# nihalsid/single-view-3d-reconstruction

Measured on AMD Instinct MI355X. Metric: query-points/sec fwd+bwd (128^3 grid, 50k pts), higher is better.
Workload: dtype f32

## Files before the change

include/svr_hip.h:

```cpp
#ifndef SVR_HIP_H
#define SVR_HIP_H

#include <stdint.h>

#ifdef __cplusplus
extern "C" {
#endif

#define SVR_OK 0
#define SVR_E_BADARG (-1)
#define SVR_E_BADSHAPE (-2)
#define SVR_E_ALIGN (-3)
#define SVR_E_UNSUPPORTED (-4)
#define SVR_E_IO (-5)
#define SVR_E_NOTFOUND (-6)

#define SVR_MAX_LEVELS 6

int svr_version(void);
const char *svr_last_error(void);

typedef struct svr_pull_plan {
  const uint32_t *keys;
  const void *recs;
// ... 183 lines not shown
int64_t svr_conv3d_bwd_data_f16x3_workspace(int32_t Ci, int32_t Co);
int svr_conv3d_k3_bwd_data_f16x3(const float *dout, const float *W, float *din, int32_t B, int32_t D,
                                 int32_t H, int32_t Wd, int32_t Ci, int32_t Co, int epilogue,
                                 const float *mask, const uint32_t *amax_dout, uint32_t *amax_din,
                                 void *workspace, void *stream);
int svr_conv3d_k3_bwd_weight_f16x3(const float *in, const float *dout, float *dW, float *db, int32_t B,
                                   int32_t D, int32_t H, int32_t W, int32_t Ci, int32_t Co, int32_t param_layout,
                                   const uint32_t *amax_dout, void *workspace, void *stream);
#define SVR_CONV_FWD_F16X3 0
#define SVR_CONV_BWD_DATA_F16X3S 1
#define SVR_CONV_BWD_DATA_BF16X3 2
#define SVR_CONV_FWD_BF16X6 3
int svr_conv3d_k3_variant(int32_t op, int32_t B, int32_t D, int32_t H, int32_t Wd, int32_t Ci, int32_t Co, int32_t *ck,
                          int32_t *tn, int32_t *vt, int32_t *persistent, int64_t *workgroup_rows);

int64_t svr_bn_stats_workspace(int64_t rows, int32_t C);
int svr_bn_stats(const float *x, double *stats, int64_t rows , int32_t C,
                 void *workspace, void *stream);
int svr_bn_stats_finalize(const float *x, double *stats, const float *gamma, const float *beta, float *running_mean,
                          float *running_var, float *scale_shift, float *mean_f32, int64_t rows, int32_t C,
                          float eps, float momentum, void *workspace, void *stream);
int svr_bn_finalize_parts(const double *part, int32_t blocks, double *stats, const float *gamma, const float *beta,
                          float *running_mean, float *running_var, float *scale_shift, float *mean_f32, int64_t rows,
                          int32_t C, float eps, float momentum, void *stream);
int svr_bn_finalize(const double *stats, const float *gamma, const float *beta, float *running_mean,
                    float *running_var, float *scale_shift, float *mean_f32, int64_t rows,
                    int32_t C, float eps, float momentum, int training, void *stream);
int svr_bn_apply_pool(const float *x, const float *scale_shift, float *y, float *pooled,
                      uint8_t *argmax, int32_t B, int32_t D, int32_t H, int32_t W, int32_t C,
                      void *stream);
// ... 119 lines not shown
```

single-view-3d-reconstruction_amd/_lib.py:

```python
import ctypes as C
import os

_HERE = os.path.dirname(os.path.abspath(__file__))
LIB_PATH = os.path.join(_HERE, "lib", "libsvr_hip.so")

SVR_MAX_LEVELS = 6
EPI_NONE, EPI_BIAS, EPI_BIAS_RELU, EPI_MASK = 0, 1, 2, 3

P = C.c_void_p
I32, I64, F32 = C.c_int32, C.c_int64, C.c_float


class Conv2dDesc(C.Structure):
    _fields_ = [("src0", P), ("src1", P), ("B", I32), ("H", I32), ("W", I32), ("C0", I32), ("C1", I32), ("k", I32),
                ("stride", I32), ("act", I32), ("upsample", I32)]


class PullPlan(C.Structure):
    _fields_ = [("keys", P), ("recs", P), ("heads", P), ("n_items", I64)]


class Level(C.Structure):
    _fields_ = [("vol", P), ("gvol", P), ("C", I32), ("D", I32), ("H", I32), ("W", I32), ("col", I32), ("order", P),
                ("item_order", P), ("plan", C.POINTER(PullPlan))]
# ... 70 lines not shown
    "svr_conv3d_fwd_f16x3_stats_blocks": (I32, [I32, I32, I32, I32, I32, I32]),
    "svr_conv3d_k3_fwd_f16x3_stats": (C.c_int, [P, P, P, P, P, I32, I32, I32, I32, I32, I32, C.c_int, P, P]),
    "svr_conv3d_bwd_data_bf16x3_workspace": (I64, [I32, I32]),
    "svr_conv3d_k3_bwd_data_bf16x3": (C.c_int, [P, P, P, I32, I32, I32, I32, I32, I32, C.c_int, P, P, P]),
    "svr_conv3d_c1_fwd_stats_workspace": (I64, [I32, I32, I32, I32, I32]),
    "svr_conv3d_c1_fwd_stats": (C.c_int, [P, P, P, P, P, I32, I32, I32, I32, I32, C.c_int, P, P]),
    "svr_conv3d_k3_bwd_weight_workspace": (I64, [I32, I32, I32, I32, I32, I32]),
    "svr_conv3d_k3_bwd_weight": (C.c_int, [P, P, P, P, I32, I32, I32, I32, I32, I32, P, P]),
    "svr_conv3d_k3_bwd_weight_bf16x3_workspace": (I64, [I32, I32, I32, I32, I32, I32]),
    "svr_conv3d_k3_bwd_weight_bf16x3": (C.c_int, [P, P, P, P, I32, I32, I32, I32, I32, I32, P, P]),
    "svr_conv3d_k3_bwd_weight_bf16x3_param": (C.c_int, [P, P, P, P, I32, I32, I32, I32, I32, I32, P, P]),
    "svr_conv3d_bwd_data_f16x3_workspace": (I64, [I32, I32]),
    "svr_conv3d_k3_bwd_data_f16x3": (C.c_int, [P, P, P, I32, I32, I32, I32, I32, I32, C.c_int, P, P, P, P, P]),
    "svr_conv3d_k3_bwd_weight_f16x3": (C.c_int, [P, P, P, P, I32, I32, I32, I32, I32, I32, I32, P, P, P]),
    "svr_conv3d_k3_variant": (C.c_int, [I32, I32, I32, I32, I32, I32, I32, P, P, P, P, P]),
    "svr_bn_stats_workspace": (I64, [I64, I32]),
    "svr_bn_stats": (C.c_int, [P, P, I64, I32, P, P]),
    "svr_bn_stats_finalize": (C.c_int, [P, P, P, P, P, P, P, P, I64, I32, F32, F32, P, P]),
    "svr_bn_finalize_parts": (C.c_int, [P, I32, P, P, P, P, P, P, P, I64, I32, F32, F32, P]),
    "svr_bn_finalize": (C.c_int, [P, P, P, P, P, P, P, I64, I32, F32, F32, C.c_int, P]),
    "svr_bn_apply_pool": (C.c_int, [P, P, P, P, P, I32, I32, I32, I32, I32, P]),
    "svr_bn_bwd_reduce": (C.c_int, [P, P, P, P, P, P, P, I32, I32, I32, I32, I32, P, P]),
    "svr_bn_bwd_apply": (C.c_int, [P, P, P, P, P, P, P, P, P, P, P, I32, I32, I32, I32, I32, C.c_int, P, P]),
    "svr_stage1_supported": (I32, [I32, I32, I32, I32, I32]),
    "svr_stage1_workspace": (I64, [I32, I32, I32, I32]),
    "svr_stage1_fwd": (C.c_int, [P, P, P, P, P, P, P, P, P, P, P, P, P, I32, I32, I32, I32, I32, F32, F32, C.c_int, C.c_int, P, P]),
    "svr_stage1_bwd": (C.c_int, [P, P, P, P, P, P, P, P, P, P, P, P, P, P, I32, I32, I32, I32, I32, C.c_int, C.c_int, P, P]),
    "svr_conv2d_im2col": (C.c_int, [C.POINTER(Conv2dDesc), P, P]),
    "svr_conv2d_col2im": (C.c_int, [C.POINTER(Conv2dDesc), P, P, P, P, P]),
    "svr_conv2d_small_supported": (C.c_int, [I32, I32, I32]),
# ... 74 lines not shown
```

single-view-3d-reconstruction_amd/build.py:

```python
import os
import subprocess
import sys

HERE = os.path.dirname(os.path.abspath(__file__))
CSRC = os.path.join(HERE, "csrc")
INCLUDE = os.path.join(os.path.dirname(HERE), "include")
LIBDIR = os.path.join(HERE, "lib")
LIB = os.path.join(LIBDIR, "libsvr_hip.so")

SOURCES = {
    "capi.cpp": [],
    "gather.hip": ["-ffp-contract=off"],
    "gather_fc0.hip": ["-ffp-contract=off"],
    "sort.hip": [],
    "gemm.hip": [],
    "gemm_bf16x3.hip": [],
    "gemm_bf16x6.hip": [],
    "gemm_f16x3.hip": [],
    "conv3d.hip": [],
    "conv3d_bf16.hip": [],
    "conv3d_bwdw_bf16.hip": [],
    "bn_pool.hip": [],
    "stage1.hip": [],
    "projection.hip": ["-ffp-contract=off"],
    "bf16_path.hip": ["-ffp-contract=off"],
    "mesh_occupancy.hip": ["-ffp-contract=off"],
    "marching_cubes.hip": ["-ffp-contract=off"],
    "mesh_eval.hip": ["-ffp-contract=off"],
    "sample_io.hip": [],
    "conv2d.hip": [],
    "conv2d_igemm.hip": [],
}
COMMON = ["-O3", "-fPIC", "--offload-arch=gfx950", "-munsafe-fp-atomics", "-std=c++17", "-I" + INCLUDE, "-I" + CSRC,
          "-Rpass-analysis=kernel-resource-usage"]


# ... 80 lines not shown
```

single-view-3d-reconstruction_amd/csrc/conv3d_bf16.hip:

```cpp
#include "common.h"
#include <cstdlib>
#include "f16x3.h"

using namespace svr;

namespace {

typedef __bf16 bf16x8 __attribute__((ext_vector_type(8)));
typedef __bf16 bf16x2 __attribute__((ext_vector_type(2)));
typedef float f32x16 __attribute__((ext_vector_type(16)));

struct ConvShape {
  int B, D, H, W, Ci, Co;
};

constexpr int BRZ = 4, BRY = 4, BRX = 8;
constexpr int HLZ = BRZ + 2, HLY = BRY + 2, HLX = BRX + 2, HLV = HLZ * HLY * HLX;

__device__ __forceinline__ void split2(float x0, float x1, uint32_t &hi, uint32_t &mid) {
  f32x2 v = {x0, x1};
  bf16x2 h = __builtin_convertvector(v, bf16x2);
  hi = __builtin_bit_cast(uint32_t, h);
  f32x2 r = {x0 - __uint_as_float(hi << 16), x1 - __uint_as_float(hi & 0xffff0000u)};
  bf16x2 m = __builtin_convertvector(r, bf16x2);
  mid = __builtin_bit_cast(uint32_t, m);
}

__device__ __forceinline__ void split3(float x0, float x1, uint32_t &hi, uint32_t &mid, uint32_t &lo) {
  split2(x0, x1, hi, mid);
  f32x2 r = {(x0 - __uint_as_float(hi << 16)) - __uint_as_float(mid << 16),
             (x1 - __uint_as_float(hi & 0xffff0000u)) - __uint_as_float(mid & 0xffff0000u)};
  bf16x2 l = __builtin_convertvector(r, bf16x2);
  lo = __builtin_bit_cast(uint32_t, l);
}

constexpr int HP = 12;
template <int SL>
__device__ __forceinline__ int slot_dw(int row, int sub) {
  static_assert(SL == 2 || SL == 4, "16- or 32-channel chunks");
  const int g = SL == 2 ? (row >> 3) & 1 : (row >> 2) & 3;
  return (row * SL + (sub ^ g)) * 4;
// ... 3 lines not shown

__device__ __forceinline__ bf16x8 read_frag(const uint32_t *p) {
  union { uint4 q; bf16x8 v; } f;
  f.q = *reinterpret_cast<const uint4 *>(p);
  return f.v;
}

__device__ __forceinline__ f16x8 read_frag_h(const uint32_t *p) {
  union { uint4 q; f16x8 v; } f;
  f.q = *reinterpret_cast<const uint4 *>(p);
  return f.v;
}

__global__ void pack_fwd_planes_f16_kernel(const float *__restrict__ W, const uint32_t *__restrict__ amax,
                                           uint16_t *__restrict__ p0, uint16_t *__restrict__ p1, int Ci, int Co) {
  int idx = blockIdx.x * blockDim.x + threadIdx.x;
  if (idx >= 27 * Co * (Ci / 2)) return;
  const int ci = (idx % (Ci / 2)) * 2;
  const int co = (idx / (Ci / 2)) % Co;
  const int tap = idx / ((Ci / 2) * Co);
  const float sc = w_scale(amax[0], false);
  const float w0 = W[((size_t)co * Ci + ci) * 27 + tap] * sc, w1 = W[((size_t)co * Ci + ci + 1) * 27 + tap] * sc;
  const uint32_t hi = pack_f16(w0, w1);
  const f32x2 h = unpack_f16(hi);
  const size_t o = ((size_t)tap * Co + co) * Ci + ci;
  *reinterpret_cast<uint32_t *>(p0 + o) = hi;
  *reinterpret_cast<uint32_t *>(p1 + o) = pack_f16(w0 - h.x, w1 - h.y);
}

__global__ void pack_bwd_planes_kernel(const float *__restrict__ W, uint16_t *__restrict__ hi, uint16_t *__restrict__ mid,
                                       int Ci, int Co) {
  int idx = blockIdx.x * blockDim.x + threadIdx.x;
  if (idx >= 27 * Ci * (Co / 2)) return;
  const int co = (idx % (Co / 2)) * 2;
  const int ci = (idx / (Co / 2)) % Ci;
  const int tp = idx / ((Co / 2) * Ci);
  uint32_t h, m;
  split2(W[((size_t)co * Ci + ci) * 27 + (26 - tp)], W[((size_t)(co + 1) * Ci + ci) * 27 + (26 - tp)], h, m);
  const size_t o = ((size_t)tp * Ci + ci) * Co + co;
  *reinterpret_cast<uint32_t *>(hi + o) = h;
  *reinterpret_cast<uint32_t *>(mid + o) = m;
}

__global__ void pack_bwd_planes_f16_kernel(const float *__restrict__ W, const uint32_t *__restrict__ amax,
                                           uint16_t *__restrict__ p0, uint16_t *__restrict__ p1, int Ci, int Co) {
  int idx = blockIdx.x * blockDim.x + threadIdx.x;
  if (idx >= 27 * Ci * (Co / 2)) return;
  const int co = (idx % (Co / 2)) * 2;
  const int ci = (idx / (Co / 2)) % Ci;
  const int tp = idx / ((Co / 2) * Ci);
  const float sc = w_scale(amax[0], false);
  const float w0 = W[((size_t)co * Ci + ci) * 27 + (26 - tp)] * sc, w1 = W[((size_t)(co + 1) * Ci + ci) * 27 + (26 - tp)] * sc;
  const uint32_t hi = pack_f16(w0, w1);
  const f32x2 h = unpack_f16(hi);
  const size_t o = ((size_t)tp * Ci + ci) * Co + co;
  *reinterpret_cast<uint32_t *>(p0 + o) = hi;
  *reinterpret_cast<uint32_t *>(p1 + o) = pack_f16(w0 - h.x, w1 - h.y);
}

__global__ void pack_fwd_planes_kernel(const float *__restrict__ W, uint16_t *__restrict__ p0, uint16_t *__restrict__ p1,
                                       uint16_t *__restrict__ p2, int Ci, int Co) {
  int idx = blockIdx.x * blockDim.x + threadIdx.x;
  if (idx >= 27 * Co * (Ci / 2)) return;
  const int ci = (idx % (Ci / 2)) * 2;
  const int co = (idx / (Ci / 2)) % Co;
  const int tap = idx / ((Ci / 2) * Co);
  uint32_t h, m, l;
  split3(W[((size_t)co * Ci + ci) * 27 + tap], W[((size_t)co * Ci + ci + 1) * 27 + tap], h, m, l);
  const size_t o = ((size_t)tap * Co + co) * Ci + ci;
  *reinterpret_cast<uint32_t *>(p0 + o) = h;
  *reinterpret_cast<uint32_t *>(p1 + o) = m;
  *reinterpret_cast<uint32_t *>(p2 + o) = l;
// ... 755 lines not shown
```

single-view-3d-reconstruction_amd/csrc/gemm_bf16x3.hip:

```cpp
#include "common.h"
#include "conv2d_virt.h"
#include "f16x3.h"

using namespace svr;

namespace svr {
void colsum_launch(const float *Y, int64_t ldy, float *out, float *part, int64_t M, int64_t N, hipStream_t s);
int64_t colsum_workspace_floats(int64_t M, int64_t N);
}

namespace {

typedef __bf16 bf16x8 __attribute__((ext_vector_type(8)));
typedef __bf16 bf16x2 __attribute__((ext_vector_type(2)));
typedef float f32x2 __attribute__((ext_vector_type(2)));
typedef float f32x16 __attribute__((ext_vector_type(16)));

constexpr int XK = 32;
constexpr int XLD = 40;
constexpr int XLW = XLD / 2;

__device__ __forceinline__ void split2(float x0, float x1, uint32_t &hi, uint32_t &mid) {
  f32x2 v = {x0, x1};
  bf16x2 h = __builtin_convertvector(v, bf16x2);
  hi = __builtin_bit_cast(uint32_t, h);
  f32x2 r = {x0 - __uint_as_float(hi << 16), x1 - __uint_as_float(hi & 0xffff0000u)};
  bf16x2 m = __builtin_convertvector(r, bf16x2);
  mid = __builtin_bit_cast(uint32_t, m);
}

template <int ROWS, int NT, bool F16 = false>
struct RowKLoader {
  static constexpr int R = ROWS * 8 / NT;
  const float *rowp[R];
  float4 v[R];
  float sy = 1.f;
  __device__ __forceinline__ RowKLoader(const float *src, int64_t ld, int64_t row0, int64_t nrows) {
    const int t = threadIdx.x;
#pragma unroll
    for (int i = 0; i < R; ++i) {
      int64_t r = row0 + (t >> 3) + (NT / 8) * i;
      r = r < nrows ? r : nrows - 1;
      rowp[i] = src + r * ld + (t & 7) * 4;
    }
// ... 200 lines not shown
__device__ __forceinline__ void foreach_acc(f32x16 (&acc)[2][2], F f) {
  const int lane = threadIdx.x & 63, wave = threadIdx.x >> 6;
  const int wr = wave / WC, wc = wave % WC;
#pragma unroll
  for (int i = 0; i < 2; ++i)
#pragma unroll
    for (int j = 0; j < 2; ++j) {
      const int col = wc * 64 + j * 32 + (lane & 31);
#pragma unroll
      for (int r = 0; r < 16; ++r) f(wr * 64 + i * 32 + (r & 3) + 8 * (r >> 2) + 4 * (lane >> 5), col, acc[i][j][r]);
    }
}

__global__ void pack_planes_kernel(const float *__restrict__ W, int64_t ldw, uint16_t *__restrict__ hi,
                                   uint16_t *__restrict__ mid, int64_t N, int64_t K) {
  int64_t idx = (int64_t)blockIdx.x * blockDim.x + threadIdx.x;
  if (idx >= K * (N / 2)) return;
  int64_t k = idx / (N / 2), n = (idx % (N / 2)) * 2;
  uint32_t h, m;
  split2(W[n * ldw + k], W[(n + 1) * ldw + k], h, m);
  *reinterpret_cast<uint32_t *>(hi + k * N + n) = h;
  *reinterpret_cast<uint32_t *>(mid + k * N + n) = m;
}

constexpr int NN_TM = 128, NN_TN = 128, NN_CLD = NN_TN + 4;
template <bool F16>
__global__ __launch_bounds__(256, 3) void linear_nn_x3_kernel(const float *__restrict__ dY, int64_t lddy,
                                                           const uint16_t *__restrict__ Wh,
                                                           const uint16_t *__restrict__ Wm, float *__restrict__ dX,
                                                           int64_t lddx, const float *__restrict__ mask, int64_t ldmask,
                                                           int64_t M, int64_t N, int64_t K, const uint32_t *__restrict__ amax_w,
                                                           const uint32_t *__restrict__ amax_dy, uint32_t *__restrict__ amax_dx) {
  using G = Geo<2, 2>;
  static_assert(G::LDS_DWORDS >= (NN_TM / 2) * NN_CLD, "half the epilogue tile must fit the staging buffer");
  __shared__ __attribute__((aligned(16))) uint32_t lds[G::LDS_DWORDS];
  const int64_t nct = cdiv(K, NN_TN), lidx = xcd_logical(blockIdx.x, gridDim.x);
  if (lidx >= nct * cdiv(M, NN_TM)) return;
// ... 42 lines not shown
          __builtin_nontemporal_store(nt4{v.x, v.y, v.z, v.w}, reinterpret_cast<nt4 *>(dX + m * lddx + c));
        } else {
          *reinterpret_cast<float4 *>(dX + m * lddx + c) = v;
        }
      }
    }
    __syncthreads();
  }
  if constexpr (F16) {
    if (amax_dx) svr_amax_publish(amax_dx, vmax);
  }
}

__global__ void pack_planes_f16_kernel(const float *__restrict__ W, int64_t ldw, const uint32_t *__restrict__ amax,
                                       uint16_t *__restrict__ hi, uint16_t *__restrict__ lo, int64_t N, int64_t K) {
  int64_t idx = (int64_t)blockIdx.x * blockDim.x + threadIdx.x;
  if (idx >= K * (N / 2)) return;
  const int64_t k = idx / (N / 2), n = (idx % (N / 2)) * 2;
  const float sc = w_scale(amax[0], false);
  const float w0 = W[n * ldw + k] * sc, w1 = W[(n + 1) * ldw + k] * sc;
  const uint32_t h = pack_f16(w0, w1);
  const f32x2 hf = unpack_f16(h);
  *reinterpret_cast<uint32_t *>(hi + k * N + n) = h;
  *reinterpret_cast<uint32_t *>(lo + k * N + n) = pack_f16(w0 - hf.x, w1 - hf.y);
}

constexpr int TN_TM = 128, TN_TN = 128;
__global__ __launch_bounds__(256) void linear_tn_x3_kernel(const uint16_t *__restrict__ dYh,
                                                           const uint16_t *__restrict__ dYm, int64_t Mpad,
                                                           const float *__restrict__ X, int64_t ldx,
                                                           float *__restrict__ slab, int64_t M, int64_t N, int64_t K,
                                                           int64_t rows_per_split, int splits) {
  using G = Geo<2, 2>;
  __shared__ __attribute__((aligned(16))) uint32_t lds[G::LDS_DWORDS];
  const int64_t tk = cdiv(K, TN_TN), tiles = tk * cdiv(N, TN_TM), lidx = xcd_logical(blockIdx.x, gridDim.x);
  if (lidx >= tiles * splits) return;
  const int64_t split = lidx / tiles, tile = lidx % tiles;
  const int64_t tn = cdiv(N, TN_TM);
  const int64_t i0 = (tile % tn) * TN_TM, j0 = (tile / tn) * TN_TN;
// ... 501 lines not shown
```

single-view-3d-reconstruction_amd/csrc/gemm_f16x3.hip:

```cpp
#include "common.h"
#include "f16x3.h"
#include <algorithm>

using namespace svr;

namespace {

typedef float f32x16 __attribute__((ext_vector_type(16)));

constexpr int YK = 16;
constexpr int YLW = 8;
constexpr int TM = 128;
constexpr int APLANE = TM * YLW;

__device__ __forceinline__ int slot_dw(int row, int h) { return (row * 2 + (h ^ ((row >> 3) & 1))) * 4; }

__device__ __forceinline__ f16x8 read_frag(const uint32_t *plane, int row, int lh) {
  union { uint4 q; f16x8 v; } f;
  f.q = *reinterpret_cast<const uint4 *>(plane + slot_dw(row, lh));
  return f.v;
}

__device__ __forceinline__ int64_t wplane_index(int64_t k, int plane, int64_t n, int64_t N) {
  return (((k >> 4) * 2 + plane) * N + n) * 16 + (k & 15);
}
__global__ void split_w_kernel(const float *__restrict__ W, int64_t ldw, const uint32_t *__restrict__ amax,
                               uint16_t *__restrict__ p0, int64_t N, int64_t K, int transposed) {
  int64_t idx = (int64_t)blockIdx.x * blockDim.x + threadIdx.x;
  if (idx >= N * (K / 2)) return;
  const int64_t n = idx / (K / 2), k = (idx % (K / 2)) * 2;
  const float sc = w_scale(amax[0], false);
  const float w0 = (transposed ? W[k * ldw + n] : W[n * ldw + k]) * sc, w1 = (transposed ? W[(k + 1) * ldw + n] : W[n * ldw + k + 1]) * sc;
  const uint32_t hi = pack_f16(w0, w1);
  const f32x2 h = unpack_f16(hi);
  *reinterpret_cast<uint32_t *>(p0 + wplane_index(k, 0, n, N)) = hi;
  *reinterpret_cast<uint32_t *>(p0 + wplane_index(k, 1, n, N)) = pack_f16(w0 - h.x, w1 - h.y);
}


template <int TN, int NX, int SCHED, bool BWD = false>
__global__ __launch_bounds__(2 * TN, 1024 / (2 * TN) >= 4 ? 3 : 2) void linear_nt_h3_kernel(
    const float *__restrict__ X, int64_t ldx, const uint16_t *__restrict__ W0,
    const uint32_t *__restrict__ amax, const float *__restrict__ bias, float *__restrict__ Y, int64_t ldy, int64_t M,
    int64_t N, int64_t K, int relu, const uint32_t *__restrict__ amax_x, const float *__restrict__ mask, int64_t ldm,
    uint32_t *__restrict__ amax_y) {
  constexpr int NT = 2 * TN, BPLANE = TN * YLW, XPT = 512 / NT, STAGE = 2 * APLANE + 2 * BPLANE;
  __shared__ __attribute__((aligned(16))) uint32_t lds[2 * STAGE];
  const int t = threadIdx.x;
  const int lane = t & 63, wave = t >> 6;
  const int wr = wave / (TN / 64), wc = wave % (TN / 64);
  const int l31 = lane & 31, lh = lane >> 5;
// ... 295 lines not shown
```

single-view-3d-reconstruction_amd/ops.py:

```python
import ctypes as C
import os

import torch

from . import _lib
from .arena import alloc as _alloc
from ._lib import EPI_BIAS, EPI_BIAS_RELU, EPI_MASK, EPI_NONE, GatherDesc, check


def _stream():
    return C.c_void_p(torch.cuda.current_stream().cuda_stream)


def _p(t):
    if t is None:
        return C.c_void_p(0)
    if not t.is_cuda:
        raise RuntimeError("svr_amd ops need GPU tensors (the HIP path has no CPU fallback)")
    if not t.is_contiguous():
        raise RuntimeError("svr_amd ops need contiguous tensors")
    return C.c_void_p(t.data_ptr())


def _f32(*ts):
# ... 435 lines not shown
          "fc_out_fwd_bf16")
    return out


FORWARD_GEMM = "f16x3"


class PreparedWeights:

    def __init__(self):
        self._ws = {}
        self._valid = {}
        self._events = []
        self.ready = None
        self._waited = set()

    def _buf(self, key, nbytes, device):
        t = self._ws.get(key)
        if t is None or t.numel() < nbytes or t.device != device:
            t = self._ws[key] = torch.empty(nbytes, device=device, dtype=torch.uint8)
        return t

    def begin(self):
        self._valid.clear()
        self._events = []
        self._waited = set()

    def add_conv(self, w, which="both"):
        _f32(w)
        Co, Ci = w.shape[0], w.shape[1]
        l = _lib.lib()
        z = C.c_void_p(0)
        fwd, bwd = which in ("fwd", "both"), which in ("bwd", "both")
        if fwd and FORWARD_CONV == "f16x3" and Ci % 16 == 0:
            ws = self._buf(("cf", w.data_ptr()), l.svr_conv3d_fwd_f16x3_workspace(Ci, Co), w.device)
            check(l.svr_conv3d_k3_fwd_f16x3(z, _p(w), z, z, 0, 0, 0, 0, Ci, Co, EPI_NONE, _p(ws), _stream()), "conv3d_fwd_f16x3 prepare")
            self._valid[("cf", w.data_ptr())] = (w._version, len(self._events))
        if bwd and BACKWARD_CONV == "bf16x3" and Ci % 2 == 0 and Co % 16 == 0:
            ws = self._buf(("cb", w.data_ptr()), l.svr_conv3d_bwd_data_bf16x3_workspace(Ci, Co), w.device)
            check(l.svr_conv3d_k3_bwd_data_bf16x3(z, _p(w), z, 0, 0, 0, 0, Ci, Co, EPI_NONE, z, _p(ws), _stream()),
                  "conv3d_bwd_data_bf16x3 prepare")
            self._valid[("cb", w.data_ptr())] = (w._version, len(self._events))
        if bwd and BACKWARD_CONV == "f16x3s" and Ci % 2 == 0 and Co % 16 == 0:
            ws = self._buf(("cbh", w.data_ptr()), l.svr_conv3d_bwd_data_f16x3_workspace(Ci, Co), w.device)
            check(l.svr_conv3d_k3_bwd_data_f16x3(z, _p(w), z, 0, 0, 0, 0, Ci, Co, EPI_NONE, z, z, z, _p(ws), _stream()),
                  "conv3d_bwd_data_f16x3 prepare")
            self._valid[("cbh", w.data_ptr())] = (w._version, len(self._events))

    def add_linear(self, w, which="both"):
        _f32(w)
        N, K = w.shape
        assert w.stride(1) == 1
        l = _lib.lib()
        z = C.c_void_p(0)
        fwd, bwd = which in ("fwd", "both"), which in ("bwd", "both")
        if fwd and FORWARD_GEMM == "f16x3" and K % 16 == 0:
            ws = self._buf(("lf", w.data_ptr()), l.svr_linear_fwd_f16x3_workspace(N, K), w.device)
            check(l.svr_linear_fwd_f16x3(z, 0, C.c_void_p(w.data_ptr()), w.stride(0), z, z, 0, 0, N, K, EPI_NONE, _p(ws), _stream()),
                  "linear_fwd_f16x3 prepare")
            self._valid[("lf", w.data_ptr())] = (w._version, len(self._events))
        if bwd and BACKWARD_GEMM == "bf16x3" and N % 32 == 0 and K % 4 == 0:
            ws = self._buf(("lb", w.data_ptr()), l.svr_linear_bwd_data_bf16x3_workspace(N, K), w.device)
            check(l.svr_linear_bwd_data_bf16x3(z, 0, C.c_void_p(w.data_ptr()), w.stride(0), z, 0, 0, N, K, EPI_NONE, z, 0, _p(ws),
                                               _stream()), "linear_bwd_data_bf16x3 prepare")
            self._valid[("lb", w.data_ptr())] = (w._version, len(self._events))
        if bwd and BACKWARD_GEMM == "f16x3s" and N % 16 == 0:
            ws = self._buf(("lbh", w.data_ptr()), l.svr_linear_bwd_data_f16x3_workspace(N, K), w.device)
            check(l.svr_linear_bwd_data_f16x3(z, 0, C.c_void_p(w.data_ptr()), w.stride(0), z, 0, 0, N, K, EPI_NONE, z, 0, z, z,
                                              _p(ws), _stream()), "linear_bwd_data_f16x3 prepare")
            self._valid[("lbh", w.data_ptr())] = (w._version, len(self._events))

    def mark(self, stream):
        ev = torch.cuda.Event()
        ev.record(stream)
        self._events.append(ev)

    def finish(self, stream):
        self.mark(stream)
        self.ready = self._events[-1]

    def invalidate(self):
        self._valid.clear()

    def lookup(self, kind, w):
        key = (kind, w.data_ptr())
        ver, idx = self._valid.get(key, (-1, 0))
        if ver != w._version or idx >= len(self._events):
# ... 754 lines not shown
```

Baseline: 25.94 million.

## Batch weight split/pack preparation into one multi-item kernel launch pair

Result: no change. 25.85 million (-0.4%).

```diff
diff --git a/include/svr_hip.h b/include/svr_hip.h
--- a/include/svr_hip.h
+++ b/include/svr_hip.h
@@ -221,6 +221,16 @@
 int svr_conv3d_k3_variant(int32_t op, int32_t B, int32_t D, int32_t H, int32_t Wd, int32_t Ci, int32_t Co, int32_t *ck,
                           int32_t *tn, int32_t *vt, int32_t *persistent, int64_t *workgroup_rows);
 
+#define SVR_PREP_MAX_ITEMS 32
+#define SVR_PREP_CONV_FWD_F16X3 0
+#define SVR_PREP_CONV_BWD_F16X3S 1
+#define SVR_PREP_CONV_BWD_BF16X3 2
+#define SVR_PREP_LINEAR_FWD_F16X3 3
+#define SVR_PREP_LINEAR_BWD_F16X3S 4
+#define SVR_PREP_LINEAR_BWD_BF16X3 5
+int svr_weights_prepare_many(int32_t n, const int32_t *kind, const float *const *W, const int64_t *ldw, const int32_t *rows,
+                             const int32_t *cols, void *const *workspace, uint32_t *amax_scratch, void *stream);
+
 int64_t svr_bn_stats_workspace(int64_t rows, int32_t C);
 int svr_bn_stats(const float *x, double *stats, int64_t rows , int32_t C,
                  void *workspace, void *stream);
diff --git a/single-view-3d-reconstruction_amd/_lib.py b/single-view-3d-reconstruction_amd/_lib.py
--- a/single-view-3d-reconstruction_amd/_lib.py
+++ b/single-view-3d-reconstruction_amd/_lib.py
@@ -6,6 +6,9 @@
 
 SVR_MAX_LEVELS = 6
 EPI_NONE, EPI_BIAS, EPI_BIAS_RELU, EPI_MASK = 0, 1, 2, 3
+PREP_CONV_FWD_F16X3, PREP_CONV_BWD_F16X3S, PREP_CONV_BWD_BF16X3 = 0, 1, 2
+PREP_LINEAR_FWD_F16X3, PREP_LINEAR_BWD_F16X3S, PREP_LINEAR_BWD_BF16X3 = 3, 4, 5
+PREP_MAX_ITEMS = 32
 
 P = C.c_void_p
 I32, I64, F32 = C.c_int32, C.c_int64, C.c_float
@@ -108,6 +111,7 @@
     "svr_conv3d_k3_bwd_data_f16x3": (C.c_int, [P, P, P, I32, I32, I32, I32, I32, I32, C.c_int, P, P, P, P, P]),
     "svr_conv3d_k3_bwd_weight_f16x3": (C.c_int, [P, P, P, P, I32, I32, I32, I32, I32, I32, I32, P, P, P]),
     "svr_conv3d_k3_variant": (C.c_int, [I32, I32, I32, I32, I32, I32, I32, P, P, P, P, P]),
+    "svr_weights_prepare_many": (C.c_int, [I32, P, P, P, P, P, P, P, P]),
     "svr_bn_stats_workspace": (I64, [I64, I32]),
     "svr_bn_stats": (C.c_int, [P, P, I64, I32, P, P]),
     "svr_bn_stats_finalize": (C.c_int, [P, P, P, P, P, P, P, P, I64, I32, F32, F32, P, P]),
diff --git a/single-view-3d-reconstruction_amd/build.py b/single-view-3d-reconstruction_amd/build.py
--- a/single-view-3d-reconstruction_amd/build.py
+++ b/single-view-3d-reconstruction_amd/build.py
@@ -20,6 +20,7 @@
     "conv3d.hip": [],
     "conv3d_bf16.hip": [],
     "conv3d_bwdw_bf16.hip": [],
+    "prepare_many.hip": [],
     "bn_pool.hip": [],
     "stage1.hip": [],
     "projection.hip": ["-ffp-contract=off"],
diff --git a/single-view-3d-reconstruction_amd/csrc/conv3d_bf16.hip b/single-view-3d-reconstruction_amd/csrc/conv3d_bf16.hip
--- a/single-view-3d-reconstruction_amd/csrc/conv3d_bf16.hip
+++ b/single-view-3d-reconstruction_amd/csrc/conv3d_bf16.hip
@@ -1,13 +1,13 @@
 #include "common.h"
 #include <cstdlib>
 #include "f16x3.h"
+#include "weight_prep.h"
 
 using namespace svr;
 
 namespace {
 
 typedef __bf16 bf16x8 __attribute__((ext_vector_type(8)));
-typedef __bf16 bf16x2 __attribute__((ext_vector_type(2)));
 typedef float f32x16 __attribute__((ext_vector_type(16)));
 
 struct ConvShape {
@@ -16,15 +16,6 @@
 
 constexpr int BRZ = 4, BRY = 4, BRX = 8;
 constexpr int HLZ = BRZ + 2, HLY = BRY + 2, HLX = BRX + 2, HLV = HLZ * HLY * HLX;
-
-__device__ __forceinline__ void split2(float x0, float x1, uint32_t &hi, uint32_t &mid) {
-  f32x2 v = {x0, x1};
-  bf16x2 h = __builtin_convertvector(v, bf16x2);
-  hi = __builtin_bit_cast(uint32_t, h);
-  f32x2 r = {x0 - __uint_as_float(hi << 16), x1 - __uint_as_float(hi & 0xffff0000u)};
-  bf16x2 m = __builtin_convertvector(r, bf16x2);
-  mid = __builtin_bit_cast(uint32_t, m);
-}
 
 __device__ __forceinline__ void split3(float x0, float x1, uint32_t &hi, uint32_t &mid, uint32_t &lo) {
   split2(x0, x1, hi, mid);
@@ -58,48 +49,15 @@
 
 __global__ void pack_fwd_planes_f16_kernel(const float *__restrict__ W, const uint32_t *__restrict__ amax,
                                            uint16_t *__restrict__ p0, uint16_t *__restrict__ p1, int Ci, int Co) {
-  int idx = blockIdx.x * blockDim.x + threadIdx.x;
-  if (idx >= 27 * Co * (Ci / 2)) return;
-  const int ci = (idx % (Ci / 2)) * 2;
-  const int co = (idx / (Ci / 2)) % Co;
-  const int tap = idx / ((Ci / 2) * Co);
-  const float sc = w_scale(amax[0], false);
-  const float w0 = W[((size_t)co * Ci + ci) * 27 + tap] * sc, w1 = W[((size_t)co * Ci + ci + 1) * 27 + tap] * sc;
-  const uint32_t hi = pack_f16(w0, w1);
-  const f32x2 h = unpack_f16(hi);
-  const size_t o = ((size_t)tap * Co + co) * Ci + ci;
-  *reinterpret_cast<uint32_t *>(p0 + o) = hi;
-  *reinterpret_cast<uint32_t *>(p1 + o) = pack_f16(w0 - h.x, w1 - h.y);
-}
-
+  prep_conv_fwd_f16(W, amax, p0, p1, Ci, Co, blockIdx.x * blockDim.x + threadIdx.x);
+}
 __global__ void pack_bwd_planes_kernel(const float *__restrict__ W, uint16_t *__restrict__ hi, uint16_t *__restrict__ mid,
                                        int Ci, int Co) {
-  int idx = blockIdx.x * blockDim.x + threadIdx.x;
-  if (idx >= 27 * Ci * (Co / 2)) return;
-  const int co = (idx % (Co / 2)) * 2;
-  const int ci = (idx / (Co / 2)) % Ci;
-  const int tp = idx / ((Co / 2) * Ci);
-  uint32_t h, m;
-  split2(W[((size_t)co * Ci + ci) * 27 + (26 - tp)], W[((size_t)(co + 1) * Ci + ci) * 27 + (26 - tp)], h, m);
-  const size_t o = ((size_t)tp * Ci + ci) * Co + co;
-  *reinterpret_cast<uint32_t *>(hi + o) = h;
-  *reinterpret_cast<uint32_t *>(mid + o) = m;
-}
-
+  prep_conv_bwd_bf16(W, hi, mid, Ci, Co, blockIdx.x * blockDim.x + threadIdx.x);
+}
 __global__ void pack_bwd_planes_f16_kernel(const float *__restrict__ W, const uint32_t *__restrict__ amax,
                                            uint16_t *__restrict__ p0, uint16_t *__restrict__ p1, int Ci, int Co) {
-  int idx = blockIdx.x * blockDim.x + threadIdx.x;
-  if (idx >= 27 * Ci * (Co / 2)) return;
-  const int co = (idx % (Co / 2)) * 2;
-  const int ci = (idx / (Co / 2)) % Ci;
-  const int tp = idx / ((Co / 2) * Ci);
-  const float sc = w_scale(amax[0], false);
-  const float w0 = W[((size_t)co * Ci + ci) * 27 + (26 - tp)] * sc, w1 = W[((size_t)(co + 1) * Ci + ci) * 27 + (26 - tp)] * sc;
-  const uint32_t hi = pack_f16(w0, w1);
-  const f32x2 h = unpack_f16(hi);
-  const size_t o = ((size_t)tp * Ci + ci) * Co + co;
-  *reinterpret_cast<uint32_t *>(p0 + o) = hi;
-  *reinterpret_cast<uint32_t *>(p1 + o) = pack_f16(w0 - h.x, w1 - h.y);
+  prep_conv_bwd_f16(W, amax, p0, p1, Ci, Co, blockIdx.x * blockDim.x + threadIdx.x);
 }
 
 __global__ void pack_fwd_planes_kernel(const float *__restrict__ W, uint16_t *__restrict__ p0, uint16_t *__restrict__ p1,
diff --git a/single-view-3d-reconstruction_amd/csrc/gemm_bf16x3.hip b/single-view-3d-reconstruction_amd/csrc/gemm_bf16x3.hip
--- a/single-view-3d-reconstruction_amd/csrc/gemm_bf16x3.hip
+++ b/single-view-3d-reconstruction_amd/csrc/gemm_bf16x3.hip
@@ -1,6 +1,7 @@
 #include "common.h"
 #include "conv2d_virt.h"
 #include "f16x3.h"
+#include "weight_prep.h"
 
 using namespace svr;
 
@@ -12,22 +13,12 @@
 namespace {
 
 typedef __bf16 bf16x8 __attribute__((ext_vector_type(8)));
-typedef __bf16 bf16x2 __attribute__((ext_vector_type(2)));
 typedef float f32x2 __attribute__((ext_vector_type(2)));
 typedef float f32x16 __attribute__((ext_vector_type(16)));
 
 constexpr int XK = 32;
 constexpr int XLD = 40;
 constexpr int XLW = XLD / 2;
-
-__device__ __forceinline__ void split2(float x0, float x1, uint32_t &hi, uint32_t &mid) {
-  f32x2 v = {x0, x1};
-  bf16x2 h = __builtin_convertvector(v, bf16x2);
-  hi = __builtin_bit_cast(uint32_t, h);
-  f32x2 r = {x0 - __uint_as_float(hi << 16), x1 - __uint_as_float(hi & 0xffff0000u)};
-  bf16x2 m = __builtin_convertvector(r, bf16x2);
-  mid = __builtin_bit_cast(uint32_t, m);
-}
 
 template <int ROWS, int NT, bool F16 = false>
 struct RowKLoader {
@@ -258,13 +249,7 @@
 
 __global__ void pack_planes_kernel(const float *__restrict__ W, int64_t ldw, uint16_t *__restrict__ hi,
                                    uint16_t *__restrict__ mid, int64_t N, int64_t K) {
-  int64_t idx = (int64_t)blockIdx.x * blockDim.x + threadIdx.x;
-  if (idx >= K * (N / 2)) return;
-  int64_t k = idx / (N / 2), n = (idx % (N / 2)) * 2;
-  uint32_t h, m;
-  split2(W[n * ldw + k], W[(n + 1) * ldw + k], h, m);
-  *reinterpret_cast<uint32_t *>(hi + k * N + n) = h;
-  *reinterpret_cast<uint32_t *>(mid + k * N + n) = m;
+  prep_linear_bwd_bf16(W, ldw, hi, mid, N, K, (int64_t)blockIdx.x * blockDim.x + threadIdx.x);
 }
 
 constexpr int NN_TM = 128, NN_TN = 128, NN_CLD = NN_TN + 4;
@@ -337,15 +322,7 @@
 
 __global__ void pack_planes_f16_kernel(const float *__restrict__ W, int64_t ldw, const uint32_t *__restrict__ amax,
                                        uint16_t *__restrict__ hi, uint16_t *__restrict__ lo, int64_t N, int64_t K) {
-  int64_t idx = (int64_t)blockIdx.x * blockDim.x + threadIdx.x;
-  if (idx >= K * (N / 2)) return;
-  const int64_t k = idx / (N / 2), n = (idx % (N / 2)) * 2;
-  const float sc = w_scale(amax[0], false);
-  const float w0 = W[n * ldw + k] * sc, w1 = W[(n + 1) * ldw + k] * sc;
-  const uint32_t h = pack_f16(w0, w1);
-  const f32x2 hf = unpack_f16(h);
-  *reinterpret_cast<uint32_t *>(hi + k * N + n) = h;
-  *reinterpret_cast<uint32_t *>(lo + k * N + n) = pack_f16(w0 - hf.x, w1 - hf.y);
+  prep_linear_bwd_f16(W, ldw, amax, hi, lo, N, K, (int64_t)blockIdx.x * blockDim.x + threadIdx.x);
 }
 
 constexpr int TN_TM = 128, TN_TN = 128;
diff --git a/single-view-3d-reconstruction_amd/csrc/gemm_f16x3.hip b/single-view-3d-reconstruction_amd/csrc/gemm_f16x3.hip
--- a/single-view-3d-reconstruction_amd/csrc/gemm_f16x3.hip
+++ b/single-view-3d-reconstruction_amd/csrc/gemm_f16x3.hip
@@ -1,5 +1,6 @@
 #include "common.h"
 #include "f16x3.h"
+#include "weight_prep.h"
 #include <algorithm>
 
 using namespace svr;
@@ -21,20 +22,9 @@
   return f.v;
 }
 
-__device__ __forceinline__ int64_t wplane_index(int64_t k, int plane, int64_t n, int64_t N) {
-  return (((k >> 4) * 2 + plane) * N + n) * 16 + (k & 15);
-}
 __global__ void split_w_kernel(const float *__restrict__ W, int64_t ldw, const uint32_t *__restrict__ amax,
                                uint16_t *__restrict__ p0, int64_t N, int64_t K, int transposed) {
-  int64_t idx = (int64_t)blockIdx.x * blockDim.x + threadIdx.x;
-  if (idx >= N * (K / 2)) return;
-  const int64_t n = idx / (K / 2), k = (idx % (K / 2)) * 2;
-  const float sc = w_scale(amax[0], false);
-  const float w0 = (transposed ? W[k * ldw + n] : W[n * ldw + k]) * sc, w1 = (transposed ? W[(k + 1) * ldw + n] : W[n * ldw + k + 1]) * sc;
-  const uint32_t hi = pack_f16(w0, w1);
-  const f32x2 h = unpack_f16(hi);
-  *reinterpret_cast<uint32_t *>(p0 + wplane_index(k, 0, n, N)) = hi;
-  *reinterpret_cast<uint32_t *>(p0 + wplane_index(k, 1, n, N)) = pack_f16(w0 - h.x, w1 - h.y);
+  prep_linear_f16(W, ldw, amax, p0, N, K, transposed, (int64_t)blockIdx.x * blockDim.x + threadIdx.x);
 }
 
 
diff --git a/single-view-3d-reconstruction_amd/csrc/prepare_many.hip b/single-view-3d-reconstruction_amd/csrc/prepare_many.hip
--- /dev/null
+++ b/single-view-3d-reconstruction_amd/csrc/prepare_many.hip
@@ -0,0 +1,123 @@
+#include "common.h"
+#include "weight_prep.h"
+#include <algorithm>
+
+using namespace svr;
+
+namespace {
+
+enum { K_CONV_FWD_F16, K_CONV_BWD_F16, K_CONV_BWD_BF16, K_LIN_FWD_F16, K_LIN_BWD_F16_NN, K_LIN_BWD_F16_T, K_LIN_BWD_BF16 };
+
+struct PrepItem {
+  const float *W;
+  uint32_t *amax;
+  uint16_t *p0, *p1;
+  int64_t ldw;
+  int kind, rows, cols;
+};
+struct PrepTable {
+  PrepItem it[SVR_PREP_MAX_ITEMS];
+};
+static_assert(sizeof(PrepTable) <= 4096, "kernel arguments passed by value");
+
+__device__ __forceinline__ bool is_conv(int kind) { return kind <= K_CONV_BWD_BF16; }
+
+__global__ __launch_bounds__(256) void prep_amax_many_kernel(const PrepTable T, uint32_t *__restrict__ scratch) {
+  const PrepItem L = T.it[blockIdx.y];
+  if (!L.amax) return;
+  const int64_t cols = is_conv(L.kind) ? (int64_t)27 * L.rows * L.cols : L.cols;
+  const int64_t rows = is_conv(L.kind) ? 1 : L.rows, ld = is_conv(L.kind) ? cols : L.ldw;
+  float m = 0.f;
+  if (ld == cols && (((uintptr_t)L.W) & 15) == 0) {
+    const int64_t n = rows * cols, n4 = n >> 2;
+    for (int64_t i = (int64_t)blockIdx.x * 256 + threadIdx.x; i < n4; i += (int64_t)gridDim.x * 256) {
+      const float4 v = reinterpret_cast<const float4 *>(L.W)[i];
+      m = fmaxf(fmaxf(m, fmaxf(fabsf(v.x), fabsf(v.y))), fmaxf(fabsf(v.z), fabsf(v.w)));
+    }
+    if (blockIdx.x == 0 && threadIdx.x < (n & 3)) m = fmaxf(m, fabsf(L.W[(n4 << 2) + threadIdx.x]));
+  } else {
+    for (int64_t i = (int64_t)blockIdx.x * 256 + threadIdx.x; i < rows * cols; i += (int64_t)gridDim.x * 256)
+      m = fmaxf(m, fabsf(L.W[(i / cols) * ld + i % cols]));
+  }
+  svr_amax_publish(scratch + blockIdx.y, m);
+}
+
+__global__ __launch_bounds__(256) void prep_split_many_kernel(const PrepTable T, const uint32_t *__restrict__ scratch) {
+  const PrepItem L = T.it[blockIdx.y];
+  const uint32_t *amax = scratch + blockIdx.y;
+  if (L.amax && blockIdx.x == 0 && threadIdx.x == 0) L.amax[0] = amax[0];
+  const int64_t pairs = (is_conv(L.kind) ? 27 : 1) * (int64_t)L.rows * L.cols / 2;
+  for (int64_t idx = (int64_t)blockIdx.x * 256 + threadIdx.x; idx < pairs; idx += (int64_t)gridDim.x * 256) {
+    switch (L.kind) {
+      case K_CONV_FWD_F16: prep_conv_fwd_f16(L.W, amax, L.p0, L.p1, L.cols, L.rows, (int)idx); break;
+      case K_CONV_BWD_F16: prep_conv_bwd_f16(L.W, amax, L.p0, L.p1, L.cols, L.rows, (int)idx); break;
+      case K_CONV_BWD_BF16: prep_conv_bwd_bf16(L.W, L.p0, L.p1, L.cols, L.rows, (int)idx); break;
+      case K_LIN_FWD_F16: prep_linear_f16(L.W, L.ldw, amax, L.p0, L.rows, L.cols, 0, idx); break;
+      case K_LIN_BWD_F16_T: prep_linear_f16(L.W, L.ldw, amax, L.p0, L.cols, L.rows, 1, idx); break;
+      case K_LIN_BWD_F16_NN: prep_linear_bwd_f16(L.W, L.ldw, amax, L.p0, L.p1, L.rows, L.cols, idx); break;
+      default: prep_linear_bwd_bf16(L.W, L.ldw, L.p0, L.p1, L.rows, L.cols, idx); break;
+    }
+  }
+}
+
+}
+
+extern "C" int svr_weights_prepare_many(int32_t n, const int32_t *kind, const float *const *W, const int64_t *ldw, const int32_t *rows,
+                                        const int32_t *cols, void *const *workspace, uint32_t *amax_scratch, void *stream) {
+  SVR_CHECK(n >= 1 && n <= SVR_PREP_MAX_ITEMS && kind && W && ldw && rows && cols && workspace && amax_scratch, SVR_E_BADARG,
+            "weights_prepare_many: 1..%d items, no null pointers", SVR_PREP_MAX_ITEMS);
+  PrepTable T{};
+  int64_t maxpairs = 0, maxnumel = 0;
+  for (int i = 0; i < n; ++i) {
+    SVR_CHECK(W[i] && workspace[i] && rows[i] > 0 && cols[i] > 0, SVR_E_BADARG, "weights_prepare_many: item %d", i);
+    const int64_t R = rows[i], Cc = cols[i];
+    PrepItem &L = T.it[i];
+    L.W = W[i], L.ldw = ldw[i], L.rows = rows[i], L.cols = cols[i];
+    uint32_t *amax = (uint32_t *)(((uintptr_t)workspace[i] + 255) & ~(uintptr_t)255);
+    uint16_t *scaled = (uint16_t *)(amax + 64), *plain = (uint16_t *)(((uintptr_t)workspace[i] + 15) & ~(uintptr_t)15);
+    const bool conv = kind[i] == SVR_PREP_CONV_FWD_F16X3 || kind[i] == SVR_PREP_CONV_BWD_F16X3S || kind[i] == SVR_PREP_CONV_BWD_BF16X3;
+    const int64_t ps = (conv ? 27 : 1) * R * Cc;
+    SVR_CHECK(ps < (1LL << 31), SVR_E_UNSUPPORTED, "weights_prepare_many: item %d has %ld elements", i, (long)ps);
+    switch (kind[i]) {
+      case SVR_PREP_CONV_FWD_F16X3:
+        SVR_CHECK(Cc % 16 == 0, SVR_E_UNSUPPORTED, "weights_prepare_many: item %d: conv forward needs Ci %% 16 == 0 (Ci=%d)", i, cols[i]);
+        L.kind = K_CONV_FWD_F16, L.amax = amax, L.p0 = scaled, L.p1 = scaled + ps;
+        break;
+      case SVR_PREP_CONV_BWD_F16X3S:
+      case SVR_PREP_CONV_BWD_BF16X3:
+        SVR_CHECK(R % 16 == 0 && Cc % 2 == 0, SVR_E_UNSUPPORTED,
+                  "weights_prepare_many: item %d: conv backward-data needs Co %% 16 == 0, Ci even (Ci=%d Co=%d)", i, cols[i], rows[i]);
+        if (kind[i] == SVR_PREP_CONV_BWD_F16X3S) L.kind = K_CONV_BWD_F16, L.amax = amax, L.p0 = scaled, L.p1 = scaled + ps;
+        else L.kind = K_CONV_BWD_BF16, L.amax = nullptr, L.p0 = plain, L.p1 = plain + ps;
+        break;
+      case SVR_PREP_LINEAR_FWD_F16X3:
+        SVR_CHECK(Cc % 16 == 0 && L.ldw >= Cc, SVR_E_BADSHAPE, "weights_prepare_many: item %d: linear forward needs K %% 16 == 0 (K=%d)", i, cols[i]);
+        L.kind = K_LIN_FWD_F16, L.amax = amax, L.p0 = scaled, L.p1 = nullptr;
+        break;
+      case SVR_PREP_LINEAR_BWD_F16X3S:
+        SVR_CHECK(R % 16 == 0 && L.ldw >= Cc, SVR_E_BADSHAPE, "weights_prepare_many: item %d: linear backward-data needs N %% 16 == 0 (N=%d)", i, rows[i]);
+        L.amax = amax, L.p0 = scaled;
+        if (R % 32 == 0 && Cc % 4 == 0) L.kind = K_LIN_BWD_F16_NN, L.p1 = scaled + ps;
+        else L.kind = K_LIN_BWD_F16_T, L.p1 = nullptr;
+        break;
+      case SVR_PREP_LINEAR_BWD_BF16X3:
+        SVR_CHECK(R % 32 == 0 && Cc % 4 == 0 && L.ldw >= Cc, SVR_E_BADSHAPE,
+                  "weights_prepare_many: item %d: need N %% 32 == 0, K %% 4 == 0 (N=%d K=%d)", i, rows[i], cols[i]);
+        L.kind = K_LIN_BWD_BF16, L.amax = nullptr, L.p0 = plain, L.p1 = plain + ps;
+        break;
+      default:
+        SVR_CHECK(false, SVR_E_BADARG, "weights_prepare_many: item %d: kind %d", i, kind[i]);
+    }
+    maxpairs = std::max(maxpairs, ps / 2);
+    if (L.amax) maxnumel = std::max(maxnumel, ps);
+  }
+  hipStream_t s = (hipStream_t)stream;
+  if (maxnumel) {
+    (void)hipMemsetAsync(amax_scratch, 0, (size_t)n * sizeof(uint32_t), s);
+    hipLaunchKernelGGL(prep_amax_many_kernel, dim3((unsigned)std::min<int64_t>(cdiv(maxnumel, 4096), 128), (unsigned)n), dim3(256), 0, s, T,
+                       amax_scratch);
+  }
+  hipLaunchKernelGGL(prep_split_many_kernel, dim3((unsigned)std::min<int64_t>(cdiv(maxpairs, 256), 1024), (unsigned)n), dim3(256), 0, s, T,
+                     (const uint32_t *)amax_scratch);
+  return launch_status("weights_prepare_many");
+}
diff --git a/single-view-3d-reconstruction_amd/csrc/weight_prep.h b/single-view-3d-reconstruction_amd/csrc/weight_prep.h
--- /dev/null
+++ b/single-view-3d-reconstruction_amd/csrc/weight_prep.h
@@ -0,0 +1,98 @@
+#pragma once
+#include "f16x3.h"
+
+namespace {
+
+typedef __bf16 bf16x2 __attribute__((ext_vector_type(2)));
+
+__device__ __forceinline__ void split2(float x0, float x1, uint32_t &hi, uint32_t &mid) {
+  f32x2 v = {x0, x1};
+  bf16x2 h = __builtin_convertvector(v, bf16x2);
+  hi = __builtin_bit_cast(uint32_t, h);
+  f32x2 r = {x0 - __uint_as_float(hi << 16), x1 - __uint_as_float(hi & 0xffff0000u)};
+  bf16x2 m = __builtin_convertvector(r, bf16x2);
+  mid = __builtin_bit_cast(uint32_t, m);
+}
+
+__device__ __forceinline__ void prep_conv_fwd_f16(const float *__restrict__ W, const uint32_t *__restrict__ amax,
+                                                  uint16_t *__restrict__ p0, uint16_t *__restrict__ p1, int Ci, int Co, int idx) {
+  if (idx >= 27 * Co * (Ci / 2)) return;
+  const int ci = (idx % (Ci / 2)) * 2;
+  const int co = (idx / (Ci / 2)) % Co;
+  const int tap = idx / ((Ci / 2) * Co);
+  const float sc = w_scale(amax[0], false);
+  const float w0 = W[((size_t)co * Ci + ci) * 27 + tap] * sc, w1 = W[((size_t)co * Ci + ci + 1) * 27 + tap] * sc;
+  const uint32_t hi = pack_f16(w0, w1);
+  const f32x2 h = unpack_f16(hi);
+  const size_t o = ((size_t)tap * Co + co) * Ci + ci;
+  *reinterpret_cast<uint32_t *>(p0 + o) = hi;
+  *reinterpret_cast<uint32_t *>(p1 + o) = pack_f16(w0 - h.x, w1 - h.y);
+}
+
+__device__ __forceinline__ void prep_conv_bwd_bf16(const float *__restrict__ W, uint16_t *__restrict__ hi, uint16_t *__restrict__ mid,
+                                                   int Ci, int Co, int idx) {
+  if (idx >= 27 * Ci * (Co / 2)) return;
+  const int co = (idx % (Co / 2)) * 2;
+  const int ci = (idx / (Co / 2)) % Ci;
+  const int tp = idx / ((Co / 2) * Ci);
+  uint32_t h, m;
+  split2(W[((size_t)co * Ci + ci) * 27 + (26 - tp)], W[((size_t)(co + 1) * Ci + ci) * 27 + (26 - tp)], h, m);
+  const size_t o = ((size_t)tp * Ci + ci) * Co + co;
+  *reinterpret_cast<uint32_t *>(hi + o) = h;
+  *reinterpret_cast<uint32_t *>(mid + o) = m;
+}
+
+__device__ __forceinline__ void prep_conv_bwd_f16(const float *__restrict__ W, const uint32_t *__restrict__ amax,
+                                                  uint16_t *__restrict__ p0, uint16_t *__restrict__ p1, int Ci, int Co, int idx) {
+  if (idx >= 27 * Ci * (Co / 2)) return;
+  const int co = (idx % (Co / 2)) * 2;
+  const int ci = (idx / (Co / 2)) % Ci;
+  const int tp = idx / ((Co / 2) * Ci);
+  const float sc = w_scale(amax[0], false);
+  const float w0 = W[((size_t)co * Ci + ci) * 27 + (26 - tp)] * sc, w1 = W[((size_t)(co + 1) * Ci + ci) * 27 + (26 - tp)] * sc;
+  const uint32_t hi = pack_f16(w0, w1);
+  const f32x2 h = unpack_f16(hi);
+  const size_t o = ((size_t)tp * Ci + ci) * Co + co;
+  *reinterpret_cast<uint32_t *>(p0 + o) = hi;
+  *reinterpret_cast<uint32_t *>(p1 + o) = pack_f16(w0 - h.x, w1 - h.y);
+}
+
+__device__ __forceinline__ int64_t wplane_index(int64_t k, int plane, int64_t n, int64_t N) {
+  return (((k >> 4) * 2 + plane) * N + n) * 16 + (k & 15);
+}
+__device__ __forceinline__ void prep_linear_f16(const float *__restrict__ W, int64_t ldw, const uint32_t *__restrict__ amax,
+                                                uint16_t *__restrict__ p0, int64_t N, int64_t K, int transposed, int64_t idx) {
+  if (idx >= N * (K / 2)) return;
+  const int64_t n = idx / (K / 2), k = (idx % (K / 2)) * 2;
+  const float sc = w_scale(amax[0], false);
+  const float w0 = (transposed ? W[k * ldw + n] : W[n * ldw + k]) * sc, w1 = (transposed ? W[(k + 1) * ldw + n] : W[n * ldw + k + 1]) * sc;
+  const uint32_t hi = pack_f16(w0, w1);
+  const f32x2 h = unpack_f16(hi);
+  *reinterpret_cast<uint32_t *>(p0 + wplane_index(k, 0, n, N)) = hi;
+  *reinterpret_cast<uint32_t *>(p0 + wplane_index(k, 1, n, N)) = pack_f16(w0 - h.x, w1 - h.y);
+}
+
+__device__ __forceinline__ void prep_linear_bwd_bf16(const float *__restrict__ W, int64_t ldw, uint16_t *__restrict__ hi,
+                                                     uint16_t *__restrict__ mid, int64_t N, int64_t K, int64_t idx) {
+  if (idx >= K * (N / 2)) return;
+  int64_t k = idx / (N / 2), n = (idx % (N / 2)) * 2;
+  uint32_t h, m;
+  split2(W[n * ldw + k], W[(n + 1) * ldw + k], h, m);
+  *reinterpret_cast<uint32_t *>(hi + k * N + n) = h;
+  *reinterpret_cast<uint32_t *>(mid + k * N + n) = m;
+}
+
+__device__ __forceinline__ void prep_linear_bwd_f16(const float *__restrict__ W, int64_t ldw, const uint32_t *__restrict__ amax,
+                                                    uint16_t *__restrict__ hi, uint16_t *__restrict__ lo, int64_t N, int64_t K,
+                                                    int64_t idx) {
+  if (idx >= K * (N / 2)) return;
+  const int64_t k = idx / (N / 2), n = (idx % (N / 2)) * 2;
+  const float sc = w_scale(amax[0], false);
+  const float w0 = W[n * ldw + k] * sc, w1 = W[(n + 1) * ldw + k] * sc;
+  const uint32_t h = pack_f16(w0, w1);
+  const f32x2 hf = unpack_f16(h);
+  *reinterpret_cast<uint32_t *>(hi + k * N + n) = h;
+  *reinterpret_cast<uint32_t *>(lo + k * N + n) = pack_f16(w0 - hf.x, w1 - hf.y);
+}
+
+}
diff --git a/single-view-3d-reconstruction_amd/ops.py b/single-view-3d-reconstruction_amd/ops.py
--- a/single-view-3d-reconstruction_amd/ops.py
+++ b/single-view-3d-reconstruction_amd/ops.py
@@ -473,6 +473,7 @@
         self._events = []
         self.ready = None
         self._waited = set()
+        self._pending = []
 
     def _buf(self, key, nbytes, device):
         t = self._ws.get(key)
@@ -483,53 +484,54 @@
     def begin(self):
         self._valid.clear()
         self._events = []
+        self._pending = []
         self._waited = set()
+
+    def _add(self, key, kind, w, ldw, rows, cols, nbytes):
+        ws = self._buf((key, w.data_ptr()), nbytes, w.device)
+        self._pending.append((kind, w, ldw, rows, cols, ws))
+        self._valid[(key, w.data_ptr())] = (w._version, len(self._events))
 
     def add_conv(self, w, which="both"):
         _f32(w)
+        assert w.is_contiguous()
         Co, Ci = w.shape[0], w.shape[1]
         l = _lib.lib()
-        z = C.c_void_p(0)
         fwd, bwd = which in ("fwd", "both"), which in ("bwd", "both")
         if fwd and FORWARD_CONV == "f16x3" and Ci % 16 == 0:
-            ws = self._buf(("cf", w.data_ptr()), l.svr_conv3d_fwd_f16x3_workspace(Ci, Co), w.device)
-            check(l.svr_conv3d_k3_fwd_f16x3(z, _p(w), z, z, 0, 0, 0, 0, Ci, Co, EPI_NONE, _p(ws), _stream()), "conv3d_fwd_f16x3 prepare")
-            self._valid[("cf", w.data_ptr())] = (w._version, len(self._events))
+            self._add("cf", _lib.PREP_CONV_FWD_F16X3, w, 0, Co, Ci, l.svr_conv3d_fwd_f16x3_workspace(Ci, Co))
         if bwd and BACKWARD_CONV == "bf16x3" and Ci % 2 == 0 and Co % 16 == 0:
-            ws = self._buf(("cb", w.data_ptr()), l.svr_conv3d_bwd_data_bf16x3_workspace(Ci, Co), w.device)
-            check(l.svr_conv3d_k3_bwd_data_bf16x3(z, _p(w), z, 0, 0, 0, 0, Ci, Co, EPI_NONE, z, _p(ws), _stream()),
-                  "conv3d_bwd_data_bf16x3 prepare")
-            self._valid[("cb", w.data_ptr())] = (w._version, len(self._events))
+            self._add("cb", _lib.PREP_CONV_BWD_BF16X3, w, 0, Co, Ci, l.svr_conv3d_bwd_data_bf16x3_workspace(Ci, Co))
         if bwd and BACKWARD_CONV == "f16x3s" and Ci % 2 == 0 and Co % 16 == 0:
-            ws = self._buf(("cbh", w.data_ptr()), l.svr_conv3d_bwd_data_f16x3_workspace(Ci, Co), w.device)
-            check(l.svr_conv3d_k3_bwd_data_f16x3(z, _p(w), z, 0, 0, 0, 0, Ci, Co, EPI_NONE, z, z, z, _p(ws), _stream()),
-                  "conv3d_bwd_data_f16x3 prepare")
-            self._valid[("cbh", w.data_ptr())] = (w._version, len(self._events))
+            self._add("cbh", _lib.PREP_CONV_BWD_F16X3S, w, 0, Co, Ci, l.svr_conv3d_bwd_data_f16x3_workspace(Ci, Co))
 
     def add_linear(self, w, which="both"):
         _f32(w)
         N, K = w.shape
         assert w.stride(1) == 1
         l = _lib.lib()
-        z = C.c_void_p(0)
         fwd, bwd = which in ("fwd", "both"), which in ("bwd", "both")
         if fwd and FORWARD_GEMM == "f16x3" and K % 16 == 0:
-            ws = self._buf(("lf", w.data_ptr()), l.svr_linear_fwd_f16x3_workspace(N, K), w.device)
-            check(l.svr_linear_fwd_f16x3(z, 0, C.c_void_p(w.data_ptr()), w.stride(0), z, z, 0, 0, N, K, EPI_NONE, _p(ws), _stream()),
-                  "linear_fwd_f16x3 prepare")
-            self._valid[("lf", w.data_ptr())] = (w._version, len(self._events))
+            self._add("lf", _lib.PREP_LINEAR_FWD_F16X3, w, w.stride(0), N, K, l.svr_linear_fwd_f16x3_workspace(N, K))
         if bwd and BACKWARD_GEMM == "bf16x3" and N % 32 == 0 and K % 4 == 0:
-            ws = self._buf(("lb", w.data_ptr()), l.svr_linear_bwd_data_bf16x3_workspace(N, K), w.device)
-            check(l.svr_linear_bwd_data_bf16x3(z, 0, C.c_void_p(w.data_ptr()), w.stride(0), z, 0, 0, N, K, EPI_NONE, z, 0, _p(ws),
-                                               _stream()), "linear_bwd_data_bf16x3 prepare")
-            self._valid[("lb", w.data_ptr())] = (w._version, len(self._events))
+            self._add("lb", _lib.PREP_LINEAR_BWD_BF16X3, w, w.stride(0), N, K, l.svr_linear_bwd_data_bf16x3_workspace(N, K))
         if bwd and BACKWARD_GEMM == "f16x3s" and N % 16 == 0:
-            ws = self._buf(("lbh", w.data_ptr()), l.svr_linear_bwd_data_f16x3_workspace(N, K), w.device)
-            check(l.svr_linear_bwd_data_f16x3(z, 0, C.c_void_p(w.data_ptr()), w.stride(0), z, 0, 0, N, K, EPI_NONE, z, 0, z, z,
-                                              _p(ws), _stream()), "linear_bwd_data_f16x3 prepare")
-            self._valid[("lbh", w.data_ptr())] = (w._version, len(self._events))
+            self._add("lbh", _lib.PREP_LINEAR_BWD_F16X3S, w, w.stride(0), N, K, l.svr_linear_bwd_data_f16x3_workspace(N, K))
+
+    def _flush(self):
+        todo, self._pending = self._pending, []
+        l = _lib.lib()
+        for g0 in range(0, len(todo), _lib.PREP_MAX_ITEMS):
+            grp = todo[g0:g0 + _lib.PREP_MAX_ITEMS]
+            n = len(grp)
+            scratch = self._buf(("amax", len(self._events), g0), 4 * _lib.PREP_MAX_ITEMS, grp[0][1].device)
+            I32A, I64A, PA = C.c_int32 * n, C.c_int64 * n, C.c_void_p * n
+            check(l.svr_weights_prepare_many(n, I32A(*[g[0] for g in grp]), PA(*[g[1].data_ptr() for g in grp]),
+                                             I64A(*[g[2] for g in grp]), I32A(*[g[3] for g in grp]), I32A(*[g[4] for g in grp]),
+                                             PA(*[g[5].data_ptr() for g in grp]), _p(scratch), _stream()), "weights_prepare_many")
 
     def mark(self, stream):
+        self._flush()
         ev = torch.cuda.Event()
         ev.record(stream)
         self._events.append(ev)
```
